# nadongjun/mirbft

Hardware: AMD Instinct MI355X
Metric: SHA-256 digests/s (request + batch digests), Actions.Hash stream (higher is better)
Workload: dtype u32

## Files before the change

### mirbft_amd/csrc/mirsha_kernels.hip

```cpp
#include <algorithm>
#include <atomic>
#include <cstdlib>
#include <cstdio>

#include <hip/hip_ext.h>

#include "mirsha_kernels.h"
#include "sha256_device.h"

namespace mirsha {

template <bool kMax>
__device__ __forceinline__ uint32_t wave_reduce(uint32_t v) {
    auto op = [](uint32_t a, uint32_t b) { return kMax ? (a > b ? a : b) : (a < b ? a : b); };
    constexpr int id = kMax ? 0 : -1;
    v = op(v, (uint32_t)__builtin_amdgcn_update_dpp(id, (int)v, 0xB1, 0xF, 0xF, false));
    v = op(v, (uint32_t)__builtin_amdgcn_update_dpp(id, (int)v, 0x4E, 0xF, 0xF, false));
    v = op(v, (uint32_t)__builtin_amdgcn_update_dpp(id, (int)v, 0x124, 0xF, 0xF, false));
    v = op(v, (uint32_t)__builtin_amdgcn_update_dpp(id, (int)v, 0x128, 0xF, 0xF, false));
    const uint32_t r0 = __builtin_amdgcn_readlane(v, 0), r1 = __builtin_amdgcn_readlane(v, 16);
    const uint32_t r2 = __builtin_amdgcn_readlane(v, 32), r3 = __builtin_amdgcn_readlane(v, 48);
    return op(op(r0, r1), op(r2, r3));
}
__device__ __forceinline__ uint32_t wave_max(uint32_t v) { return wave_reduce<true>(v); }
__device__ __forceinline__ uint32_t wave_min(uint32_t v) { return wave_reduce<false>(v); }

struct RawChunk {
    uint32_t v[5];
    uint32_t sel;
};

__device__ __forceinline__ void issue_chunk(__amdgpu_buffer_rsrc_t rsrc, uint32_t records, uint32_t o,
                                            uint32_t blk, uint32_t q, bool active, RawChunk& c) {
    const uint32_t addr = o + 64u * blk + 16u * q;
    const uint32_t a = active ? (addr & ~3u) : 0xFFFFFFE0u;
    c.sel = be_sel(addr & 3u);
    if (a + 20u <= records || !active) {
        const auto v = __builtin_amdgcn_raw_buffer_load_b128(rsrc, a, 0, 0);
        c.v[0] = v[0]; c.v[1] = v[1]; c.v[2] = v[2]; c.v[3] = v[3];
        c.v[4] = __builtin_amdgcn_raw_buffer_load_b32(rsrc, a + 16u, 0, 0);
    } else {
        asm volatile(
            "s_nop 4\n\t"
            "buffer_load_dword %0, %5, %6, 0 offen\n\t"
            "buffer_load_dword %1, %5, %6, 0 offen offset:4\n\t"
            "buffer_load_dword %2, %5, %6, 0 offen offset:8\n\t"
            "buffer_load_dword %3, %5, %6, 0 offen offset:12\n\t"
            "buffer_load_dword %4, %5, %6, 0 offen offset:16\n\t"
            "s_waitcnt vmcnt(0)"
            : "=&v"(c.v[0]), "=&v"(c.v[1]), "=&v"(c.v[2]), "=&v"(c.v[3]), "=&v"(c.v[4])
            : "v"(a), "s"(rsrc)
            : "memory");
    }
}

typedef uint32_t u32x4a4 __attribute__((ext_vector_type(4), aligned(4)));
__device__ __forceinline__ void issue_chunk_wide(const uint8_t* __restrict__ arena, uint64_t records, uint64_t o,
                                                 uint32_t blk, uint32_t q, bool active, RawChunk& c) {
    const uint64_t addr = o + 64ull * blk + 16u * q;
    const uint64_t a = addr & ~3ull;
    c.sel = be_sel((uint32_t)addr & 3u);
#pragma unroll
    for (int k = 0; k < 5; k++) c.v[k] = 0u;
    if (active) {
        const uint32_t* p = reinterpret_cast<const uint32_t*>(arena + a);
        if (a + 20u <= records) {
            const u32x4a4 v = *reinterpret_cast<const u32x4a4*>(p);
            c.v[0] = v[0]; c.v[1] = v[1]; c.v[2] = v[2]; c.v[3] = v[3];
            c.v[4] = p[4];
        } else {
#pragma unroll
            for (int k = 0; k < 5; k++)
                if (a + 4u * k + 4u <= records) c.v[k] = p[k];
        }
    }
}

__device__ __forceinline__ void pad_words(uint32_t p, uint32_t L, bool last_block, uint32_t q, uint32_t out[4]) {
    if (p + 16u > L) {
#pragma unroll
        for (int k = 0; k < 4; k++) {
            const int32_t t = (int32_t)(L - (p + 4u * k));
            const uint32_t sh = (uint32_t)t << 3;
            const uint32_t keep = ~(0xFFFFFFFFu >> sh);
            const uint32_t mark = 0x80000000u >> sh;
            const uint32_t part = (out[k] & keep) | mark;
            out[k] = t >= 4 ? out[k] : (t < 0 ? 0u : part);
        }
        if (last_block && q == 3u) {
            out[2] = L >> 29;
            out[3] = L << 3;
        }
    }
}

template <int kWords = 16>
__device__ __forceinline__ void pad_block_uniform(uint32_t w[16], uint32_t soff, uint32_t L, bool last) {
#pragma unroll
    for (int k = 0; k < kWords; k++) {
        const int32_t t = (int32_t)(L - (soff + 4u * k));
        const uint32_t sh = (uint32_t)t << 3;
        uint32_t keep = t >= 4 ? 0xFFFFFFFFu : (t <= 0 ? 0u : ~(0xFFFFFFFFu >> sh));
        uint32_t mark = (t >= 0 && t < 4) ? 0x80000000u >> sh : 0u;
        if (k >= 14 && last) {
            keep = 0u;
            mark = k == 14 ? L >> 29 : L << 3;
        }
        keep = __builtin_amdgcn_readfirstlane(keep);
        mark = __builtin_amdgcn_readfirstlane(mark);
        w[k] = (w[k] & keep) | mark;
    }
}

__device__ __forceinline__ void finish_chunk(const RawChunk& c, uint32_t p, uint32_t L, bool last_block,
                                             uint32_t q, uint32_t out[4]) {
#pragma unroll
    for (int k = 0; k < 4; k++) out[k] = be_word(c.v[k + 1], c.v[k], c.sel);
    pad_words(p, L, last_block, q, out);
}

__device__ __forceinline__ uint32_t lds_slot(uint32_t m, uint32_t q) {
    return m * 4u + (q ^ ((m >> 2) & 3u));
}

__device__ __forceinline__ void store_digest(uint8_t* out, uint32_t msg, const uint32_t st[8]) {
    uint4* d = reinterpret_cast<uint4*>(out + 32ull * msg);
    d[0] = make_uint4(__builtin_bswap32(st[0]), __builtin_bswap32(st[1]), __builtin_bswap32(st[2]),
                      __builtin_bswap32(st[3]));
    d[1] = make_uint4(__builtin_bswap32(st[4]), __builtin_bswap32(st[5]), __builtin_bswap32(st[6]),
                      __builtin_bswap32(st[7]));
}

__device__ __forceinline__ void store_digest_buf(__amdgpu_buffer_rsrc_t ors, uint32_t msg, const uint32_t st[8]) {
    __builtin_amdgcn_raw_buffer_store_b128(
        (uint32_t __attribute__((ext_vector_type(4)))){__builtin_bswap32(st[0]), __builtin_bswap32(st[1]),
                                                        __builtin_bswap32(st[2]), __builtin_bswap32(st[3])},
        ors, 32u * msg, 0, 0);
    __builtin_amdgcn_raw_buffer_store_b128(
        (uint32_t __attribute__((ext_vector_type(4)))){__builtin_bswap32(st[4]), __builtin_bswap32(st[5]),
                                                        __builtin_bswap32(st[6]), __builtin_bswap32(st[7])},
        ors, 32u * msg + 16u, 0, 0);
}

constexpr int kSc1 = 1 << 4;

__device__ __forceinline__ void store_digest_sc1(__amdgpu_buffer_rsrc_t ors, uint32_t msg, const uint32_t st[8]) {
    __builtin_amdgcn_raw_buffer_store_b128(
        (uint32_t __attribute__((ext_vector_type(4)))){__builtin_bswap32(st[0]), __builtin_bswap32(st[1]),
                                                        __builtin_bswap32(st[2]), __builtin_bswap32(st[3])},
        ors, 32u * msg, 0, kSc1);
    __builtin_amdgcn_raw_buffer_store_b128(
        (uint32_t __attribute__((ext_vector_type(4)))){__builtin_bswap32(st[4]), __builtin_bswap32(st[5]),
                                                        __builtin_bswap32(st[6]), __builtin_bswap32(st[7])},
        ors, 32u * msg + 16u, 0, kSc1);
}

constexpr uint32_t kPrioTop = 3;
__device__ __forceinline__ void progress_prio(uint32_t blk) {
    blk = (uint32_t)__builtin_amdgcn_readfirstlane((int)blk);
    const uint32_t p = blk < kPrioTop ? kPrioTop - blk : 0u;
    if (p >= 3u) __builtin_amdgcn_s_setprio(3);
    else if (p == 2u) __builtin_amdgcn_s_setprio(2);
    else if (p == 1u) __builtin_amdgcn_s_setprio(1);
    else __builtin_amdgcn_s_setprio(0);
}

constexpr uint32_t kPrioProgress = 4;
__device__ __forceinline__ void fixed_prio(uint32_t p) {
    p = (uint32_t)__builtin_amdgcn_readfirstlane((int)p);
    if (p >= 3u) __builtin_amdgcn_s_setprio(3);
    else if (p == 2u) __builtin_amdgcn_s_setprio(2);
    else if (p == 1u) __builtin_amdgcn_s_setprio(1);
    else __builtin_amdgcn_s_setprio(0);
}

constexpr uint32_t kPrioBalance = 5;
constexpr uint32_t kBalDone = 0xFFFFFFFFu;
__shared__ uint32_t g_bal_prog[4 * 16];

__device__ __forceinline__ uint32_t lds_addr(const void* p) {
    return (uint32_t)(size_t)(const __attribute__((address_space(3))) void*)p;
}
__device__ __forceinline__ uint32_t lds_load_nodma(const uint32_t* p) {
    uint32_t v;
    asm volatile("ds_read_b32 %0, %1\n\ts_waitcnt lgkmcnt(0)" : "=v"(v) : "v"(lds_addr(p)) : "memory");
    return v;
}

__shared__ uint32_t g_simd_live[4];
constexpr uint32_t kLoneSeen = 0xFFFFFFFFu;
__device__ __forceinline__ bool simd_alone(uint32_t sel) {
    if (sel == 0u || sel == kLoneSeen) return sel != 0u;
    const uint32_t n = lds_load_nodma(&g_simd_live[sel - 1u]);
    return (uint32_t)__builtin_amdgcn_readfirstlane((int)n) <= 1u;
}
__device__ __forceinline__ uint32_t bal_word() {
    uint32_t hw;
    asm volatile("s_getreg_b32 %0, hwreg(HW_REG_HW_ID)" : "=s"(hw));
    return ((hw >> 4) & 3u) * 16u + (hw & 15u);
}
__device__ __forceinline__ void balance_prio(uint32_t blk) {
    const uint32_t me = bal_word();
    __hip_atomic_store(g_bal_prog + me, blk, __ATOMIC_RELAXED, __HIP_MEMORY_SCOPE_WORKGROUP);
    const uint32_t* row = g_bal_prog + (me & ~15u);
    uint32_t ahead = 0;
#pragma unroll
    for (uint32_t k = 0; k < 16; k++)
        ahead += __hip_atomic_load(row + k, __ATOMIC_RELAXED, __HIP_MEMORY_SCOPE_WORKGROUP) < blk ? 1u : 0u;
    fixed_prio(3u - min(3u, (uint32_t)__builtin_amdgcn_readfirstlane((int)ahead)));
}
__device__ __forceinline__ void balance_done() {
    __hip_atomic_store(g_bal_prog + bal_word(), kBalDone, __ATOMIC_RELAXED, __HIP_MEMORY_SCOPE_WORKGROUP);
}

template <bool kNoYield>
__device__ __forceinline__ void hash_tile_pipelined(__amdgpu_buffer_rsrc_t rsrc, const uint32_t vo[4],
                                                    const uint32_t sel[4], uint32_t L, uint32_t min_l, bool uni,
                                                    bool tail_ok, const TailWords& tw, uint32_t wave_nb,
                                                    uint32_t loop_nb, uint32_t nb, uint32_t lane, uint4* my,
                                                    uint32_t st[8]) {
    const uint32_t q = lane & 3u;
    uint32_t nx[4][4];
    auto load_raw = [&](uint32_t blk) {
#pragma unroll
        for (int j = 0; j < 4; j++) {
            const auto v = __builtin_amdgcn_raw_buffer_load_b128(rsrc, vo[j], 64u * blk, 0);
            nx[j][0] = v[0]; nx[j][1] = v[1]; nx[j][2] = v[2]; nx[j][3] = v[3];
        }
    };
    auto write_tile = [&](uint32_t blk) {
        const uint32_t soff = 64u * blk;
        const bool pad = soff + 64u > min_l;
#pragma unroll
        for (int j = 0; j < 4; j++) {
            uint32_t wq[4];
#pragma unroll
            for (int k = 0; k < 4; k++) wq[k] = be_word(k < 3 ? nx[j][k + 1] : 0u, nx[j][k], sel[j]);
            if (pad && !uni) {
                const uint32_t Lm = (uint32_t)__shfl((int)L, 16 * j + (int)(lane >> 2), 64);
                pad_words(soff + 16u * q, Lm, blk + 1u == blocks_for_len(Lm), q, wq);
            }
            my[lds_slot(16u * j + (lane >> 2), q)] = make_uint4(wq[0], wq[1], wq[2], wq[3]);
        }
        __builtin_amdgcn_fence(__ATOMIC_RELEASE, "wavefront");
        __builtin_amdgcn_wave_barrier();
        __builtin_amdgcn_fence(__ATOMIC_ACQUIRE, "wavefront");
    };
    auto read_tile = [&](uint32_t w[16]) {
#pragma unroll
        for (int k = 0; k < 4; k++) {
            const uint4 x = my[lds_slot(lane, (uint32_t)k)];
            w[4 * k + 0] = x.x; w[4 * k + 1] = x.y; w[4 * k + 2] = x.z; w[4 * k + 3] = x.w;
        }
        __builtin_amdgcn_fence(__ATOMIC_RELEASE, "wavefront");
        __builtin_amdgcn_wave_barrier();
        __builtin_amdgcn_fence(__ATOMIC_ACQUIRE, "wavefront");
    };
    auto pad_uniform = [&](uint32_t blk, uint32_t w[16]) {
        if (64u * blk + 64u > min_l && uni) {
            uint32_t wnb;
            asm volatile("s_mov_b32 %0, %1" : "=s"(wnb) : "s"(wave_nb));
            pad_block_uniform(w, 64u * blk, min_l, wnb - blk == 1u);
        }
    };
    uint32_t w[16];
    load_raw(0u);
    write_tile(0u);
    if (1u < wave_nb) load_raw(1u);
    read_tile(w);
    for (uint32_t blk = 0; blk < loop_nb; blk++) {
        pad_uniform(blk, w);
        const bool next = blk + 1u < wave_nb;
        uint32_t wn[16];
        progress_prio(blk);
        compress_asm_hooked<kNoYield>(st, w, blk < nb, [&](int k) {
            if (k == 0 && next) {
                write_tile(blk + 1u);
                if (blk + 2u < wave_nb) load_raw(blk + 2u);
            } else if (k == 2 && next) {
                read_tile(wn);
            }
        });
#pragma unroll
        for (int i = 0; i < 16; i++) w[i] = wn[i];
    }
    if (tail_ok) {
        const uint32_t blk = wave_nb - 1u;
        pad_block_uniform<4>(w, 64u * blk, min_l, false);
        progress_prio(blk);
        if (blk < nb) compress_asm_tail(st, w, tw);
    }
}

constexpr uint32_t kTilePaused = 0, kTileDone = 1;
template <bool kLds, bool kWide, bool kFused = false, bool kPf = false, bool kNoYield = false, bool kDma = false,
          bool kDmaPipe = false, int kDiag = 0>
__device__ __forceinline__ uint32_t hash_tile(const uint8_t* __restrict__ arena, uint64_t arena_len,
                                          const uint64_t* __restrict__ off, const uint32_t* __restrict__ len,
                                          const uint32_t* __restrict__ order, uint32_t n, uint8_t* __restrict__ out,
                                          uint4* my, uint32_t t, uint32_t lane, uint32_t fprio = 0,
                                          uint32_t b0 = 0u, uint32_t b1 = 0xFFFFFFFFu, uint32_t* st_io = nullptr,
                                          uint32_t lone_sel = 0u, uint4* my2 = nullptr,
                                          unsigned long long* lone_tr = nullptr) {
    auto block_prio = [&](uint32_t blk) {
        if constexpr (kDiag == 2) {
            return;
        } else if constexpr (kFused) {
            if (fprio == kPrioBalance)
                balance_prio(blk);
            else if (fprio == kPrioProgress)
                progress_prio(blk);
            else
                fixed_prio(fprio);
        } else {
            progress_prio(blk);
        }
    };
    __builtin_amdgcn_s_setprio(3);
    const uint32_t slot = t * 64u + lane;
    const bool valid = slot < n;
    const uint32_t slot_c = valid ? slot : n - 1u;
    const uint32_t msg = order ? order[slot_c] : slot_c;
    const uint32_t L_ = len[msg];
    const uint64_t o_ = off[msg];
    const uint32_t L = valid ? L_ : 0u;
    const uint64_t o = valid ? o_ : 0u;
    const uint32_t nb = valid ? blocks_for_len(L) : 0u;
    const uint32_t max_l = wave_max(valid ? L : 0u);
    const uint32_t wave_nb = blocks_for_len(max_l);

    const uint64_t records = (arena_len + 3u) & ~3ull;
    const __amdgpu_buffer_rsrc_t rsrc =
        __builtin_amdgcn_make_buffer_rsrc((void*)arena, (short)0, (int)(uint32_t)records, 0x00020000);
    auto issue = [&](uint64_t mo, uint32_t blk, uint32_t q, bool active, RawChunk& rc) {
        if constexpr (kWide)
            issue_chunk_wide(arena, records, mo, blk, q, active, rc);
        else
            issue_chunk(rsrc, (uint32_t)records, (uint32_t)mo, blk, q, active, rc);
    };

    uint32_t st[8];
#pragma unroll
    for (int i = 0; i < 8; i++) st[i] = (st_io && b0) ? st_io[i] : kH0[i];
    const bool finished = b1 >= wave_nb;

    if constexpr (kLds && !kWide) {
        const uint32_t q = lane & 3u;
        const uint64_t reach = valid ? o + 64ull * wave_nb + 20u : 0ull;
        const bool far = __builtin_amdgcn_ballot_w64(reach > records) == 0;
        const bool aligned = __builtin_amdgcn_ballot_w64(valid && (o & 3u) != 0u) == 0;
        const uint32_t min_l = wave_min(valid ? L : 0xFFFFFFFFu);
        const bool uni = max_l == min_l;
        const int32_t u_last = (int32_t)(min_l - 64u * (wave_nb - 1u));
        const bool tail_ok = uni && u_last <= 16;
        const TailWords tw = tail_words(u_last, min_l);
        uint32_t vo[4], sel[4];
#pragma unroll
        for (int j = 0; j < 4; j++) {
            const uint32_t a = (uint32_t)__shfl((int)(uint32_t)o, 16 * j + (int)(lane >> 2), 64) + 16u * q;
            vo[j] = a & ~3u;
            sel[j] = be_sel(a & 3u);
        }
        auto stage = [&](uint32_t blk, uint32_t w[16], uint32_t ln, bool trim) {
            const uint32_t soff = 64u * blk;
            const uint32_t qq = ln & 3u;
            const bool skip = trim && soff + 16u * qq >= min_l;
            RawChunk rc[4];
            if (far && !trim) {
#pragma unroll
                for (int j = 0; j < 4; j++) {
                    const auto v = __builtin_amdgcn_raw_buffer_load_b128(rsrc, vo[j], soff, 0);
                    rc[j].v[0] = v[0]; rc[j].v[1] = v[1]; rc[j].v[2] = v[2]; rc[j].v[3] = v[3];
                    rc[j].v[4] = 0u;
                }
                if (!aligned) {
#pragma unroll
                    for (int j = 0; j < 4; j++)
                        rc[j].v[4] = __builtin_amdgcn_raw_buffer_load_b32(rsrc, vo[j], soff + 16u, 0);
                }
            } else if (far) {
#pragma unroll
                for (int j = 0; j < 4; j++) {
                    const uint32_t a = skip ? 0xFFFFFFE0u : vo[j] + soff;
                    const auto v = __builtin_amdgcn_raw_buffer_load_b128(rsrc, a, 0, 0);
                    rc[j].v[0] = v[0]; rc[j].v[1] = v[1]; rc[j].v[2] = v[2]; rc[j].v[3] = v[3];
                    rc[j].v[4] = aligned ? 0u : __builtin_amdgcn_raw_buffer_load_b32(rsrc, a + 16u, 0, 0);
                }
            } else {
#pragma unroll
                for (int j = 0; j < 4; j++)
                    issue_chunk(rsrc, (uint32_t)records, vo[j] + soff, 0u, 0u, !skip, rc[j]);
            }
            const bool pad = soff + 64u > min_l;
#pragma unroll
            for (int j = 0; j < 4; j++) {
                uint32_t wq[4];
#pragma unroll
                for (int k = 0; k < 4; k++) wq[k] = be_word(rc[j].v[k + 1], rc[j].v[k], sel[j]);
                if (pad && !uni) {
                    const uint32_t Lm = (uint32_t)__shfl((int)L, 16 * j + (int)(ln >> 2), 64);
                    pad_words(soff + 16u * qq, Lm, blk + 1u == blocks_for_len(Lm), qq, wq);
                }
                my[lds_slot(16u * j + (ln >> 2), qq)] = make_uint4(wq[0], wq[1], wq[2], wq[3]);
            }
            __builtin_amdgcn_fence(__ATOMIC_RELEASE, "wavefront");
            __builtin_amdgcn_wave_barrier();
            __builtin_amdgcn_fence(__ATOMIC_ACQUIRE, "wavefront");
#pragma unroll
            for (int k = 0; k < 4; k++) {
                const uint4 x = my[lds_slot(ln, (uint32_t)k)];
                w[4 * k + 0] = x.x; w[4 * k + 1] = x.y; w[4 * k + 2] = x.z; w[4 * k + 3] = x.w;
            }
            __builtin_amdgcn_fence(__ATOMIC_RELEASE, "wavefront");
            __builtin_amdgcn_wave_barrier();
            __builtin_amdgcn_fence(__ATOMIC_ACQUIRE, "wavefront");
        };
        const uint32_t loop_nb = tail_ok ? wave_nb - 1u : wave_nb;
        if constexpr (kPf && !kDma && !kDmaPipe) {
            if (far && aligned && b0 == 0u && finished) {
                hash_tile_pipelined<kNoYield>(rsrc, vo, sel, L, min_l, uni, tail_ok, tw, wave_nb, loop_nb, nb, lane, my,
                                              st);
                goto digest;
            }
        }
        const uint32_t loop_end = min(loop_nb, b1);
        bool dma = false;
        if constexpr (kFused || kDma || kDmaPipe) dma = far && aligned;
        if (dma) {
            const uint32_t qd = (lane & 3u) ^ ((lane >> 4) & 3u);
            uint32_t vd[4];
#pragma unroll
            for (int j = 0; j < 4; j++)
                vd[j] = (uint32_t)__shfl((int)(uint32_t)o, 16 * j + (int)(lane >> 2), 64) + 16u * qd;
            const bool deep = kFused && my2 != nullptr;
            auto tile_of = [&](uint32_t blk) { return (deep && (blk & 1u)) ? my2 : my; };
            auto issue_dma = [&](uint32_t blk) {
                if constexpr (kDiag == 1) return;
                uint4* t = tile_of(blk);
#pragma unroll
                for (int j = 0; j < 4; j++)
                    __builtin_amdgcn_raw_ptr_buffer_load_lds(
                        rsrc, (__attribute__((address_space(3))) void*)(t + 64 * j), 16, vd[j], 64u * blk, 0, 0);
            };
            const uint32_t d0 = (uint32_t)__builtin_amdgcn_readfirstlane((int)b0);
            const uint32_t d1 = (uint32_t)__builtin_amdgcn_readfirstlane((int)loop_end);
            const uint32_t dmin = (uint32_t)__builtin_amdgcn_readfirstlane((int)min_l);
            auto read_words = [&](uint32_t x[16]) {
                asm volatile("s_waitcnt vmcnt(0)" ::: "memory");
#pragma unroll
                for (int k = 0; k < 4; k++) {
                    const uint4 v = my[lds_slot(lane, (uint32_t)k)];
                    x[4 * k + 0] = v.x; x[4 * k + 1] = v.y; x[4 * k + 2] = v.z; x[4 * k + 3] = v.w;
                }
            };
            auto finish_words = [&](uint32_t blk, uint32_t x[16]) {
#pragma unroll
                for (int k = 0; k < 16; k++) x[k] = __builtin_bswap32(x[k]);
                if (64u * blk + 64u > dmin) {
                    uint32_t wnb;
                    asm volatile("s_mov_b32 %0, %1" : "=s"(wnb) : "s"(wave_nb));
                    if (uni) {
                        pad_block_uniform(x, 64u * blk, dmin, wnb - blk == 1u);
                    } else {
#pragma unroll
                        for (int k = 0; k < 4; k++)
                            pad_words(64u * blk + 16u * (uint32_t)k, L, blk + 1u == nb, (uint32_t)k, &x[4 * k]);
                    }
                }
            };
            if constexpr (kDmaPipe) {
                if (d0 < d1) {
                    uint32_t w[16];
                    issue_dma(d0);
                    read_words(w);
                    asm volatile("s_waitcnt lgkmcnt(0)" ::: "memory");
                    if (d0 + 1u < d1) issue_dma(d0 + 1u);
                    for (uint32_t blk = d0; blk < d1; blk++) {
                        finish_words(blk, w);
                        block_prio(blk);
                        const bool next = blk + 1u < d1, next2 = blk + 2u < d1;
                        uint32_t wn[16];
                        compress_asm_hooked(st, w, blk < nb, [&](int k) {
                            if (k == 2 && next) {
                                read_words(wn);
                            } else if (k == 4 && next) {
                                asm volatile("s_waitcnt lgkmcnt(0)" ::: "memory");
                                if (next2) issue_dma(blk + 2u);
                            }
                        });
#pragma unroll
                        for (int i = 0; i < 16; i++) w[i] = wn[i];
                    }
                }
            }
            if (!kDmaPipe && d0 < d1) {
                issue_dma(d0);
                if (deep && d0 + 1u < d1) issue_dma(d0 + 1u);
            }
            for (uint32_t blk = kDmaPipe ? d1 : d0; blk < d1; blk++) {
                const uint32_t soff = 64u * blk;
                if (deep && blk + 1u < d1)
                    asm volatile("s_waitcnt vmcnt(4)" ::: "memory");
                else
                    asm volatile("s_waitcnt vmcnt(0)" ::: "memory");
                if constexpr (kFused) block_prio(blk);
                uint32_t w[16];
                const uint4* tb = tile_of(blk);
#pragma unroll
                for (int k = 0; k < 4; k++) {
                    const uint4 x = tb[lds_slot(lane, (uint32_t)k)];
                    w[4 * k + 0] = x.x; w[4 * k + 1] = x.y; w[4 * k + 2] = x.z; w[4 * k + 3] = x.w;
                }
                asm volatile("s_waitcnt lgkmcnt(0)" ::: "memory");
                if (blk + (deep ? 2u : 1u) < d1) issue_dma(blk + (deep ? 2u : 1u));
#pragma unroll
                for (int k = 0; k < 16; k++) w[k] = __builtin_bswap32(w[k]);
                if (soff + 64u > dmin) {
                    uint32_t wnb;
                    asm volatile("s_mov_b32 %0, %1" : "=s"(wnb) : "s"(wave_nb));
                    if (uni) {
                        pad_block_uniform(w, soff, dmin, wnb - blk == 1u);
                    } else {
#pragma unroll
                        for (int k = 0; k < 4; k++)
                            pad_words(soff + 16u * (uint32_t)k, L, blk + 1u == nb, (uint32_t)k, &w[4 * k]);
                    }
                }
                if constexpr (!kFused) block_prio(blk);
                if constexpr (kFused) {
                    if (lone_sel != 0u && simd_alone(lone_sel)) lone_sel = kLoneSeen;
                    if (lone_sel == kLoneSeen) {
                        if (lone_tr != nullptr) {
                            if (lane == 0u) *lone_tr |= 1ull << 63 | (unsigned long long)min(blk, 1023u) << 53;
                            lone_tr = nullptr;
                        }
                        if (blk < nb) compress_asm_lat(st, w);
                    } else if (blk < nb) {
                        compress_asm(st, w);
                    }
                } else if (blk < nb) {
                    compress_asm(st, w);
                }
            }
        }
        for (uint32_t blk = dma ? loop_end : b0; blk < loop_end; blk++) {
            const uint32_t soff = 64u * blk;
            uint32_t w[16];
            stage(blk, w, lane, false);
            if (soff + 64u > min_l && uni) {
                uint32_t wnb;
                asm volatile("s_mov_b32 %0, %1" : "=s"(wnb) : "s"(wave_nb));
                pad_block_uniform(w, soff, min_l, wnb - blk == 1u);
            }
            block_prio(blk);
            if (blk < nb) compress_asm(st, w);
        }
        if (tail_ok && finished) {
            const uint32_t blk = wave_nb - 1u;
            uint32_t w[16];
            uint32_t ln;
            asm volatile("v_mov_b32 %0, %1" : "=v"(ln) : "v"(lane));
            stage(blk, w, ln, true);
            pad_block_uniform<4>(w, 64u * blk, min_l, false);
            block_prio(blk);
            if (blk < nb) compress_asm_tail(st, w, tw);
        }
    } else if constexpr (kLds) {
        const uint32_t q = lane & 3u;
        uint32_t Lj[4], nbj[4];
        uint64_t oj[4];
#pragma unroll
        for (int j = 0; j < 4; j++) {
            const int src = 16 * j + (int)(lane >> 2);
            Lj[j] = (uint32_t)__shfl((int)L, src, 64);
            oj[j] = (uint64_t)(uint32_t)__shfl((int)(uint32_t)o, src, 64);
            oj[j] |= (uint64_t)(uint32_t)__shfl((int)(uint32_t)(o >> 32), src, 64) << 32;
            nbj[j] = (uint32_t)__shfl((int)nb, src, 64);
        }
        for (uint32_t blk = 0; blk < wave_nb; blk++) {
            RawChunk rc[4];
#pragma unroll
            for (int j = 0; j < 4; j++) issue(oj[j], blk, q, blk < nbj[j], rc[j]);
#pragma unroll
            for (int j = 0; j < 4; j++) {
                uint32_t wq[4];
                finish_chunk(rc[j], 64u * blk + 16u * q, Lj[j], blk + 1u == nbj[j], q, wq);
                my[lds_slot(16u * j + (lane >> 2), q)] = make_uint4(wq[0], wq[1], wq[2], wq[3]);
            }
            __builtin_amdgcn_fence(__ATOMIC_RELEASE, "wavefront");
            __builtin_amdgcn_wave_barrier();
            __builtin_amdgcn_fence(__ATOMIC_ACQUIRE, "wavefront");
            uint32_t w[16];
#pragma unroll
            for (int k = 0; k < 4; k++) {
                const uint4 x = my[lds_slot(lane, (uint32_t)k)];
                w[4 * k + 0] = x.x; w[4 * k + 1] = x.y; w[4 * k + 2] = x.z; w[4 * k + 3] = x.w;
            }
            __builtin_amdgcn_fence(__ATOMIC_RELEASE, "wavefront");
            __builtin_amdgcn_wave_barrier();
            __builtin_amdgcn_fence(__ATOMIC_ACQUIRE, "wavefront");
            progress_prio(blk);
            if (blk < nb) compress_asm(st, w);
        }
    } else {
        for (uint32_t blk = 0; blk < wave_nb; blk++) {
            const bool active = blk < nb;
            RawChunk rc[4];
#pragma unroll
            for (int q = 0; q < 4; q++) issue(o, blk, (uint32_t)q, active, rc[q]);
            uint32_t w[16];
#pragma unroll
            for (int q = 0; q < 4; q++)
                finish_chunk(rc[q], 64u * blk + 16u * q, L, blk + 1u == nb, (uint32_t)q, &w[4 * q]);
            progress_prio(blk);
            if (active) compress_asm(st, w);
        }
    }
digest:
    if (!finished) {
#pragma unroll
        for (int i = 0; i < 8; i++) st_io[i] = st[i];
        return kTilePaused;
    }
    if (valid) {
        if constexpr (kFused) {
            const __amdgpu_buffer_rsrc_t ors =
                __builtin_amdgcn_make_buffer_rsrc((void*)out, (short)0, (int)(32u * n), 0x00020000);
            store_digest_sc1(ors, msg, st);
        } else if constexpr (kLds && !kWide) {
            const __amdgpu_buffer_rsrc_t ors =
                __builtin_amdgcn_make_buffer_rsrc((void*)out, (short)0, (int)(32u * n), 0x00020000);
            store_digest_buf(ors, msg, st);
        } else {
            store_digest(out, msg, st);
        }
    }
    return kTileDone;
}

constexpr uint32_t kMsgWaves = 1;
constexpr uint32_t kMsgOcc = 8, kTileSlots = 256;
template <bool kLds, bool kWide = false>
__global__ __launch_bounds__(64 * kMsgWaves, kWide ? 6 : kMsgOcc) void sha256_msgs_kernel(
    const uint8_t* __restrict__ arena, uint64_t arena_len, const uint64_t* __restrict__ off,
    const uint32_t* __restrict__ len, const uint32_t* __restrict__ order, uint32_t n,
    uint8_t* __restrict__ out) {
    __shared__ uint4 tile[kMsgWaves][kTileSlots];
    const uint32_t lane = threadIdx.x & 63u;
    const uint32_t wv = threadIdx.x >> 6;
    const uint32_t t = blockIdx.x * kMsgWaves + wv;
    if (t * 64u >= n) return;
    hash_tile<kLds, kWide>(arena, arena_len, off, len, order, n, out, tile[wv], t, lane);
}

constexpr uint32_t kCuLds = 96u * 1024u;
template <int kMode>
__global__ __launch_bounds__(1024, 1) void sha256_msgs_cu_kernel(const uint8_t* __restrict__ arena,
                                                                 uint64_t arena_len,
                                                                 const uint64_t* __restrict__ off,
                                                                 const uint32_t* __restrict__ len,
                                                                 const uint32_t* __restrict__ order, uint32_t n,
                                                                 uint8_t* __restrict__ out) {
    extern __shared__ uint4 cu_lds[];
    const uint32_t lane = threadIdx.x & 63u;
    const uint32_t wv = threadIdx.x >> 6;
    const uint32_t t = blockIdx.x * (blockDim.x >> 6) + wv;
    if (t * 64u >= n) return;
    hash_tile<true, false, false, true, kMode == 1, kMode == 0 || kMode >= 4, kMode == 3,
              kMode == 4 ? 1 : kMode == 5 ? 2 : 0>(arena, arena_len, off, len, order, n, out, cu_lds + 256u * wv, t,
                                                     lane);
}

__device__ __forceinline__ uint32_t ld_u32(__amdgpu_buffer_rsrc_t rs, uint32_t off, bool live);
__device__ __forceinline__ void load_digest(__amdgpu_buffer_rsrc_t rsrc, uint32_t id, bool live, uint4& x0,
                                            uint4& x1);
__device__ __forceinline__ void overlap_chain(const uint8_t* __restrict__ digests, uint32_t n_digests,
                                              const uint32_t* __restrict__ cidx, uint32_t n_entries,
                                              const uint32_t* __restrict__ cfirst, uint32_t n_lists,
                                              uint8_t* __restrict__ list_out, uint32_t g, uint32_t lane,
                                              uint32_t prio_mode) {
    __builtin_amdgcn_s_setprio(3);
    const uint32_t k = g * 64u + lane;
    const bool valid = k < n_lists;
    const uint32_t kc = valid ? k : n_lists - 1u;
    const uint32_t e0_ = cfirst[kc], e1_ = cfirst[kc + 1];
    const uint32_t e0 = valid ? e0_ : 0u;
    const uint32_t c = valid ? e1_ - e0_ : 0u;
    const uint32_t L = 32u * c;
    const uint32_t nb = valid ? blocks_for_len(L) : 0u;
    const uint32_t wave_nb = blocks_for_len(32u * wave_max(c));
    const __amdgpu_buffer_rsrc_t drs =
        __builtin_amdgcn_make_buffer_rsrc((void*)digests, (short)0, (int)(32u * n_digests), 0x00020000);
    const __amdgpu_buffer_rsrc_t irs =
        __builtin_amdgcn_make_buffer_rsrc((void*)cidx, (short)0, (int)(4u * n_entries), 0x00020000);
    uint32_t st[8];
#pragma unroll
    for (int i = 0; i < 8; i++) st[i] = kH0[i];
    uint32_t i0 = ld_u32(irs, 4u * e0, 0u < c), i1 = ld_u32(irs, 4u * (e0 + 1u), 1u < c);
    for (uint32_t blk = 0; blk < wave_nb; blk++) {
        const uint32_t d0 = 2u * blk;
        uint4 x[4];
        load_digest(drs, i0, d0 < c, x[0], x[1]);
        load_digest(drs, i1, d0 + 1u < c, x[2], x[3]);
        i0 = ld_u32(irs, 4u * (e0 + d0 + 2u), d0 + 2u < c);
        i1 = ld_u32(irs, 4u * (e0 + d0 + 3u), d0 + 3u < c);
        uint32_t w[16];
#pragma unroll
        for (int half = 0; half < 2; half++) {
            const uint32_t di = d0 + (uint32_t)half;
            const uint4 a = x[2 * half], b = x[2 * half + 1];
            w[8 * half + 0] = __builtin_bswap32(a.x) | (di == c ? 0x80000000u : 0u);
            w[8 * half + 1] = __builtin_bswap32(a.y); w[8 * half + 2] = __builtin_bswap32(a.z);
            w[8 * half + 3] = __builtin_bswap32(a.w); w[8 * half + 4] = __builtin_bswap32(b.x);
            w[8 * half + 5] = __builtin_bswap32(b.y); w[8 * half + 6] = __builtin_bswap32(b.z);
            w[8 * half + 7] = __builtin_bswap32(b.w);
        }
        if (blk + 1u == nb) {
            w[14] = L >> 29;
            w[15] = L << 3;
        }
        fixed_prio(prio_mode == 0u   ? 3u - min(3u, 4u * blk / wave_nb)
                   : prio_mode == 1u ? 3u - min(3u, blk)
                   : prio_mode == 2u ? 3u
                                     : 1u);
        if (blk < nb) compress_asm(st, w);
    }
    if (valid) {
        const __amdgpu_buffer_rsrc_t ors =
            __builtin_amdgcn_make_buffer_rsrc((void*)list_out, (short)0, (int)(32u * n_lists), 0x00020000);
        store_digest_buf(ors, k, st);
    }
}

constexpr uint32_t kOverlapOcc = 7;
__global__ __launch_bounds__(64, kOverlapOcc) void sha256_msgs_overlap_kernel(OverlapArgs a) {
    __shared__ uint4 tile[kTileSlots];
    const uint32_t lane = threadIdx.x;
    if (blockIdx.x < a.list_waves) {
        overlap_chain(a.prev_digests, a.n_req_prev, a.cidx, a.n_entries, a.cfirst, a.n_lists, a.list_out,
                      blockIdx.x, lane, a.chain_prio);
        return;
    }
    const uint32_t t = blockIdx.x - a.list_waves;
    if (t * 64u >= a.n_req) return;
    hash_tile<true, false>(a.arena, a.arena_len, a.off, a.len, a.order, a.n_req, a.req_out, tile, t, lane);
}

__global__ __launch_bounds__(kBlockThreads) void sha256_msgs_lowocc_kernel(
    const uint8_t* __restrict__ arena, uint64_t arena_len, const uint64_t* __restrict__ off,
    const uint32_t* __restrict__ len, const uint32_t* __restrict__ order, uint32_t n, uint8_t* __restrict__ out) {
    const uint32_t lane = threadIdx.x & 63u;
    const uint32_t t = blockIdx.x * kWavesPerBlock + (threadIdx.x >> 6);
    if (t * 64u >= n) return;
    const uint32_t slot = t * 64u + lane;
    const bool valid = slot < n;
    const uint32_t msg = valid ? (order ? order[slot] : slot) : 0u;
    const uint32_t L = valid ? len[msg] : 0u;
    const uint32_t o = valid ? (uint32_t)off[msg] : 0u;
    const uint32_t nb = valid ? blocks_for_len(L) : 0u;
    const uint32_t wave_nb = wave_max(nb);
    const uint32_t records = (uint32_t)((arena_len + 3u) & ~3ull);
    const __amdgpu_buffer_rsrc_t rsrc =
        __builtin_amdgcn_make_buffer_rsrc((void*)arena, (short)0, (int)records, 0x00020000);
    uint32_t st[8];
#pragma unroll
    for (int i = 0; i < 8; i++) st[i] = kH0[i];
    RawChunk cur[4];
#pragma unroll
    for (int q = 0; q < 4; q++) issue_chunk(rsrc, records, o, 0u, (uint32_t)q, 0u < nb, cur[q]);
    for (uint32_t blk = 0; blk < wave_nb; blk++) {
        RawChunk nxt[4];
#pragma unroll
        for (int q = 0; q < 4; q++) issue_chunk(rsrc, records, o, blk + 1u, (uint32_t)q, blk + 1u < nb, nxt[q]);
        uint32_t w[16];
#pragma unroll
        for (int q = 0; q < 4; q++)
            finish_chunk(cur[q], 64u * blk + 16u * q, L, blk + 1u == nb, (uint32_t)q, &w[4 * q]);
        if (blk < nb) compress_asm_lat(st, w);
#pragma unroll
        for (int q = 0; q < 4; q++) cur[q] = nxt[q];
    }
    if (valid) store_digest(out, msg, st);
}

constexpr uint32_t kPairThreads = 128;

struct PairRing {
    uint4 kw[2][16][64];
};

__device__ __forceinline__ void produce_kw(uint32_t w[16], uint4 (*slot)[64], uint32_t lane) {
#pragma unroll
    for (int q = 0; q < 16; q++) {
        uint32_t kw[4];
#pragma unroll
        for (int i = 0; i < 4; i++) {
            const int j = 4 * q + i;
            if (j >= 16) w[j & 15] += ssig1(w[(j - 2) & 15]) + w[(j - 7) & 15] + ssig0(w[(j - 15) & 15]);
            kw[i] = kK[j] + w[j & 15];
        }
        slot[q][lane] = make_uint4(kw[0], kw[1], kw[2], kw[3]);
    }
}

__device__ __forceinline__ void consume_kw(uint4 (*slot)[64], uint32_t lane, uint32_t st[8], bool live) {
    uint32_t s[8];
#pragma unroll
    for (int i = 0; i < 8; i++) s[i] = st[i];
    uint4 a = slot[0][lane], b = slot[1][lane];
#pragma unroll
    for (int c = 0; c < 8; c++) {
        uint4 na = a, nb = b;
        if (c < 7) {
            na = slot[2 * c + 2][lane];
            nb = slot[2 * c + 3][lane];
        }
        rounds_kw8_asm(s, a, b);
        a = na;
        b = nb;
    }
    if (live) {
#pragma unroll
        for (int i = 0; i < 8; i++) st[i] += s[i];
    }
}

__device__ __forceinline__ uint32_t ld_u32(__amdgpu_buffer_rsrc_t rs, uint32_t off, bool live);
__device__ __forceinline__ void load_digest(__amdgpu_buffer_rsrc_t rsrc, uint32_t id, bool live, uint4& x0,
                                            uint4& x1);

struct ArenaBlocks {
    __amdgpu_buffer_rsrc_t rsrc;
    uint32_t records, o, L, nb;
    RawChunk cur[4];
    __device__ void start(const uint8_t* arena, uint64_t arena_len, uint32_t off_, uint32_t L_, uint32_t nb_) {
        records = (uint32_t)((arena_len + 3u) & ~3ull);
        rsrc = __builtin_amdgcn_make_buffer_rsrc((void*)arena, (short)0, (int)records, 0x00020000);
        o = off_;
        L = L_;
        nb = nb_;
#pragma unroll
        for (int q = 0; q < 4; q++) issue_chunk(rsrc, records, o, 0u, (uint32_t)q, 0u < nb, cur[q]);
    }
    __device__ void block(uint32_t blk, uint32_t w[16]) {
        RawChunk nxt[4];
#pragma unroll
        for (int q = 0; q < 4; q++) issue_chunk(rsrc, records, o, blk + 1u, (uint32_t)q, blk + 1u < nb, nxt[q]);
#pragma unroll
        for (int q = 0; q < 4; q++) finish_chunk(cur[q], 64u * blk + 16u * q, L, blk + 1u == nb, (uint32_t)q, &w[4 * q]);
#pragma unroll
        for (int q = 0; q < 4; q++) cur[q] = nxt[q];
    }
};

struct ListBlocks {
    __amdgpu_buffer_rsrc_t drs, irs;
    uint32_t e0, c, L, nb;
    uint4 cur[4];
    uint32_t nx0, nx1;
    __device__ void start(const uint8_t* digests, uint32_t n_digests, const uint32_t* cidx, uint32_t n_entries,
                          uint32_t e0_, uint32_t c_, uint32_t nb_) {
        drs = __builtin_amdgcn_make_buffer_rsrc((void*)digests, (short)0, (int)(32u * n_digests), 0x00020000);
        irs = __builtin_amdgcn_make_buffer_rsrc((void*)cidx, (short)0, (int)(4u * n_entries), 0x00020000);
        e0 = e0_;
        c = c_;
        L = 32u * c;
        nb = nb_;
        nx0 = ld_u32(irs, 4u * (e0 + 2u), 2u < c);
        nx1 = ld_u32(irs, 4u * (e0 + 3u), 3u < c);
        const uint32_t i0 = ld_u32(irs, 4u * e0, 0u < c), i1 = ld_u32(irs, 4u * (e0 + 1u), 1u < c);
        load_digest(drs, i0, 0u < c, cur[0], cur[1]);
        load_digest(drs, i1, 1u < c, cur[2], cur[3]);
    }
    __device__ void block(uint32_t blk, uint32_t w[16]) {
        uint4 nxt[4];
        load_digest(drs, nx0, 2u * blk + 2u < c, nxt[0], nxt[1]);
        load_digest(drs, nx1, 2u * blk + 3u < c, nxt[2], nxt[3]);
        const uint32_t nn0 = ld_u32(irs, 4u * (e0 + 2u * blk + 4u), 2u * blk + 4u < c);
        const uint32_t nn1 = ld_u32(irs, 4u * (e0 + 2u * blk + 5u), 2u * blk + 5u < c);
#pragma unroll
        for (int half = 0; half < 2; half++) {
            const uint32_t di = 2u * blk + (uint32_t)half;
            const uint4 x0 = cur[2 * half], x1 = cur[2 * half + 1];
            w[8 * half + 0] = __builtin_bswap32(x0.x) | (di == c ? 0x80000000u : 0u);
            w[8 * half + 1] = __builtin_bswap32(x0.y); w[8 * half + 2] = __builtin_bswap32(x0.z);
            w[8 * half + 3] = __builtin_bswap32(x0.w); w[8 * half + 4] = __builtin_bswap32(x1.x);
            w[8 * half + 5] = __builtin_bswap32(x1.y); w[8 * half + 6] = __builtin_bswap32(x1.z);
            w[8 * half + 7] = __builtin_bswap32(x1.w);
        }
        if (blk + 1u == nb) {
            w[14] = L >> 29;
            w[15] = L << 3;
        }
#pragma unroll
        for (int i = 0; i < 4; i++) cur[i] = nxt[i];
        nx0 = nn0;
        nx1 = nn1;
    }
};

template <class Src>
__device__ __forceinline__ void pair_loop(Src& src, PairRing& ring, bool producer, uint32_t lane, uint32_t nb,
                                          uint32_t st[8]) {
    const uint32_t wave_nb = wave_max(nb);
#pragma unroll
    for (int i = 0; i < 8; i++) st[i] = kH0[i];
    if (producer && wave_nb) {
        uint32_t w[16];
        src.block(0u, w);
        produce_kw(w, ring.kw[0], lane);
    }
    __syncthreads();
    for (uint32_t blk = 0; blk < wave_nb; blk++) {
        if (producer) {
            if (blk + 1u < wave_nb) {
                uint32_t w[16];
                src.block(blk + 1u, w);
                produce_kw(w, ring.kw[(blk + 1u) & 1u], lane);
            }
        } else {
            consume_kw(ring.kw[blk & 1u], lane, st, blk < nb);
// ... 1256 lines not shown
```

### mirbft_amd/csrc/sha256_device.h

```cpp
#pragma once
#include <hip/hip_runtime.h>
#include <stdint.h>

#include "sha256_rounds_asm.h"

namespace mirsha {

static constexpr uint32_t kK[64] = {
    0x428a2f98u, 0x71374491u, 0xb5c0fbcfu, 0xe9b5dba5u, 0x3956c25bu, 0x59f111f1u, 0x923f82a4u,
    0xab1c5ed5u, 0xd807aa98u, 0x12835b01u, 0x243185beu, 0x550c7dc3u, 0x72be5d74u, 0x80deb1feu,
    0x9bdc06a7u, 0xc19bf174u, 0xe49b69c1u, 0xefbe4786u, 0x0fc19dc6u, 0x240ca1ccu, 0x2de92c6fu,
    0x4a7484aau, 0x5cb0a9dcu, 0x76f988dau, 0x983e5152u, 0xa831c66du, 0xb00327c8u, 0xbf597fc7u,
    0xc6e00bf3u, 0xd5a79147u, 0x06ca6351u, 0x14292967u, 0x27b70a85u, 0x2e1b2138u, 0x4d2c6dfcu,
    0x53380d13u, 0x650a7354u, 0x766a0abbu, 0x81c2c92eu, 0x92722c85u, 0xa2bfe8a1u, 0xa81a664bu,
    0xc24b8b70u, 0xc76c51a3u, 0xd192e819u, 0xd6990624u, 0xf40e3585u, 0x106aa070u, 0x19a4c116u,
    0x1e376c08u, 0x2748774cu, 0x34b0bcb5u, 0x391c0cb3u, 0x4ed8aa4au, 0x5b9cca4fu, 0x682e6ff3u,
    0x748f82eeu, 0x78a5636fu, 0x84c87814u, 0x8cc70208u, 0x90befffau, 0xa4506cebu, 0xbef9a3f7u,
    0xc67178f2u};

static constexpr uint32_t kH0[8] = {0x6a09e667u, 0xbb67ae85u, 0x3c6ef372u, 0xa54ff53au,
                                    0x510e527fu, 0x9b05688cu, 0x1f83d9abu, 0x5be0cd19u};

__device__ __forceinline__ uint32_t rotr(uint32_t x, int n) { return __builtin_rotateright32(x, n); }
__device__ __forceinline__ uint32_t xor3(uint32_t a, uint32_t b, uint32_t c) {
    return __builtin_amdgcn_bitop3_b32(a, b, c, 0x96);
}
__device__ __forceinline__ uint32_t bsig0(uint32_t x) { return xor3(rotr(x, 2), rotr(x, 13), rotr(x, 22)); }
__device__ __forceinline__ uint32_t bsig1(uint32_t x) { return xor3(rotr(x, 6), rotr(x, 11), rotr(x, 25)); }
__device__ __forceinline__ uint32_t ssig0(uint32_t x) { return xor3(rotr(x, 7), rotr(x, 18), x >> 3); }
__device__ __forceinline__ uint32_t ssig1(uint32_t x) { return xor3(rotr(x, 17), rotr(x, 19), x >> 10); }
__device__ __forceinline__ uint32_t ch(uint32_t e, uint32_t f, uint32_t g) { return g ^ (e & (f ^ g)); }
__device__ __forceinline__ uint32_t maj(uint32_t a, uint32_t b, uint32_t c) {
    return __builtin_amdgcn_bitop3_b32(a, b, c, 0xE8);
}

__device__ __forceinline__ void compress(uint32_t st[8], uint32_t w[16]) {
    uint32_t a = st[0], b = st[1], c = st[2], d = st[3];
    uint32_t e = st[4], f = st[5], g = st[6], h = st[7];
#define MIRSHA_ROUND(a, b, c, d, e, f, g, h, j)                                              \
    {                                                                                        \
        if ((j) >= 16)                                                                       \
            w[(j)&15] += ssig1(w[((j)-2) & 15]) + w[((j)-7) & 15] + ssig0(w[((j)-15) & 15]);  \
        uint32_t t1 = h + bsig1(e) + ch(e, f, g) + kK[(j)] + w[(j)&15];                      \
        d += t1;                                                                             \
        h = t1 + bsig0(a) + maj(a, b, c);                                                    \
    }
#pragma unroll
    for (int j = 0; j < 64; j += 8) {
        MIRSHA_ROUND(a, b, c, d, e, f, g, h, j + 0);
        MIRSHA_ROUND(h, a, b, c, d, e, f, g, j + 1);
        MIRSHA_ROUND(g, h, a, b, c, d, e, f, j + 2);
        MIRSHA_ROUND(f, g, h, a, b, c, d, e, j + 3);
        MIRSHA_ROUND(e, f, g, h, a, b, c, d, j + 4);
        MIRSHA_ROUND(d, e, f, g, h, a, b, c, j + 5);
        MIRSHA_ROUND(c, d, e, f, g, h, a, b, j + 6);
        MIRSHA_ROUND(b, c, d, e, f, g, h, a, j + 7);
    }
#undef MIRSHA_ROUND
    st[0] += a; st[1] += b; st[2] += c; st[3] += d;
    st[4] += e; st[5] += f; st[6] += g; st[7] += h;
}

__device__ __forceinline__ void compress_asm(uint32_t st[8], uint32_t w[16]) {
    uint32_t s[8];
#pragma unroll
    for (int i = 0; i < 8; i++) s[i] = st[i];
    rounds_asm(s, w);
#pragma unroll
    for (int i = 0; i < 8; i++) st[i] += s[i];
}

template <bool kNoYield = false, class H>
__device__ __forceinline__ void compress_asm_hooked(uint32_t st[8], uint32_t w[16], bool live, H hook) {
    uint32_t s[8];
#pragma unroll
    for (int i = 0; i < 8; i++) s[i] = st[i];
    if constexpr (kNoYield)
        rounds_asm_nonop(s, w, hook);
    else
        rounds_asm(s, w, hook);
#pragma unroll
    for (int i = 0; i < 8; i++) st[i] = live ? st[i] + s[i] : st[i];
}

__device__ __forceinline__ TailWords tail_words(int32_t u, uint32_t L) {
    auto sgpr = [](uint32_t x) { return (uint32_t)__builtin_amdgcn_readfirstlane((int)x); };
    TailWords k;
    k.c4 = u == 16 ? 0x80000000u : 0u;
    k.c14 = L >> 29;
    k.c15 = L << 3;
    k.kw4 = kK[4] + k.c4;
    k.kw14 = kK[14] + k.c14;
    k.kw15 = kK[15] + k.c15;
    k.cs16 = sgpr(ssig1(k.c14));
    k.cs17 = sgpr(ssig1(k.c15));
    k.cs19 = sgpr(ssig0(k.c4));
    k.cs29 = sgpr(ssig0(k.c14));
    k.cs30 = sgpr(ssig0(k.c15) + k.c14);
    return k;
}

__device__ __forceinline__ void compress_asm_tail(uint32_t st[8], uint32_t w[16], const TailWords& k) {
    uint32_t s[8];
#pragma unroll
    for (int i = 0; i < 8; i++) s[i] = st[i];
    rounds_asm_tail(s, w, k);
#pragma unroll
    for (int i = 0; i < 8; i++) st[i] += s[i];
}

__device__ __forceinline__ void compress_asm_lat(uint32_t st[8], uint32_t w[16]) {
    uint32_t s[8];
#pragma unroll
    for (int i = 0; i < 8; i++) s[i] = st[i];
    rounds_asm_nonop(s, w);
#pragma unroll
    for (int i = 0; i < 8; i++) st[i] += s[i];
}

__device__ __host__ __forceinline__ uint32_t blocks_for_len(uint32_t L) { return (L + 72u) >> 6; }

__device__ __forceinline__ uint32_t be_word(uint32_t hi, uint32_t lo, uint32_t sel) {
    return __builtin_amdgcn_perm(hi, lo, sel);
}
__device__ __forceinline__ uint32_t be_sel(uint32_t r) { return 0x00010203u + r * 0x01010101u; }

__device__ __forceinline__ void pad_chunk(uint32_t w[4], uint32_t p, uint32_t L, bool last_block,
                                          uint32_t q) {
#pragma unroll
    for (int k = 0; k < 4; k++) {
        const int64_t rem = (int64_t)L - (int64_t)(p + 4u * k);
        const uint32_t valid = rem <= 0 ? 0u : (rem >= 4 ? 4u : (uint32_t)rem);
        const uint32_t mask = valid == 4u ? 0xFFFFFFFFu : (valid == 0u ? 0u : ~(0xFFFFFFFFu >> (8u * valid)));
        uint32_t x = w[k] & mask;
        if (rem >= 0 && rem < 4) x |= 0x80u << (24u - 8u * (uint32_t)rem);
        w[k] = x;
    }
    if (last_block && q == 3u) {
        w[2] = L >> 29;
        w[3] = L << 3;
    }
}

}
```

Before: 5.081 billion.

## Add uniform-length dense-wave fast path skipping reductions and shuffles in LDS staging

When every valid lane in a wave has the same message length, the wave skips the min/max reductions and takes the length from the first lane. If the offsets are also contiguous and 4-byte aligned, per-lane addresses come from a scalar base instead of shuffles and ballots, and the unaligned fifth-word loads and mixed-length padding become separate cold branches. Tail-word setup is moved to where it is used and computed with scalar rotates instead of readfirstlane. This adds extra ballots/compares up front and more code paths, and it includes census asm markers, which look like instrumentation.

Measured after the change: 5.117 billion (median of 6 runs). Within noise of the previous version (+0.7%).

```diff
diff --git a/mirbft_amd/csrc/mirsha_kernels.hip b/mirbft_amd/csrc/mirsha_kernels.hip
--- a/mirbft_amd/csrc/mirsha_kernels.hip
+++ b/mirbft_amd/csrc/mirsha_kernels.hip
@@ -9,6 +9,8 @@
 #include "sha256_device.h"
 
 namespace mirsha {
+
+#define CENSUS_MARK(name) asm volatile("; census " name)
 
 template <bool kMax>
 __device__ __forceinline__ uint32_t wave_reduce(uint32_t v) {
@@ -158,10 +160,9 @@
 constexpr uint32_t kPrioTop = 3;
 __device__ __forceinline__ void progress_prio(uint32_t blk) {
     blk = (uint32_t)__builtin_amdgcn_readfirstlane((int)blk);
-    const uint32_t p = blk < kPrioTop ? kPrioTop - blk : 0u;
-    if (p >= 3u) __builtin_amdgcn_s_setprio(3);
-    else if (p == 2u) __builtin_amdgcn_s_setprio(2);
-    else if (p == 1u) __builtin_amdgcn_s_setprio(1);
+    if (blk + 3u <= kPrioTop) __builtin_amdgcn_s_setprio(3);
+    else if (blk + 2u == kPrioTop) __builtin_amdgcn_s_setprio(2);
+    else if (blk + 1u == kPrioTop) __builtin_amdgcn_s_setprio(1);
     else __builtin_amdgcn_s_setprio(0);
 }
 
@@ -326,7 +327,24 @@
     const uint32_t L = valid ? L_ : 0u;
     const uint64_t o = valid ? o_ : 0u;
     const uint32_t nb = valid ? blocks_for_len(L) : 0u;
-    const uint32_t max_l = wave_max(valid ? L : 0u);
+    uint32_t max_l, min_l = 0u;
+    [[maybe_unused]] uint32_t L0 = 0u;
+    [[maybe_unused]] bool same_len = false;
+    [[maybe_unused]] uint64_t vmask = 0;
+    if constexpr (kLds && !kWide) {
+        L0 = (uint32_t)__builtin_amdgcn_readfirstlane((int)L_);
+        vmask = __builtin_amdgcn_uicmp(slot, n, 36 );
+        same_len = (__builtin_amdgcn_uicmp(L_, L0, 33 ) & vmask) == 0;
+        if (same_len) {
+            max_l = min_l = L0;
+        } else {
+            CENSUS_MARK("off");
+            max_l = wave_max(L);
+            min_l = wave_min(valid ? L : 0xFFFFFFFFu);
+        }
+    } else {
+        max_l = wave_max(L);
+    }
     const uint32_t wave_nb = blocks_for_len(max_l);
 
     const uint64_t records = (arena_len + 3u) & ~3ull;
@@ -346,62 +364,104 @@
 
     if constexpr (kLds && !kWide) {
         const uint32_t q = lane & 3u;
-        const uint64_t reach = valid ? o + 64ull * wave_nb + 20u : 0ull;
-        const bool far = __builtin_amdgcn_ballot_w64(reach > records) == 0;
-        const bool aligned = __builtin_amdgcn_ballot_w64(valid && (o & 3u) != 0u) == 0;
-        const uint32_t min_l = wave_min(valid ? L : 0xFFFFFFFFu);
         const bool uni = max_l == min_l;
         const int32_t u_last = (int32_t)(min_l - 64u * (wave_nb - 1u));
         const bool tail_ok = uni && u_last <= 16;
-        const TailWords tw = tail_words(u_last, min_l);
+        bool far, aligned;
         uint32_t vo[4], sel[4];
-#pragma unroll
-        for (int j = 0; j < 4; j++) {
-            const uint32_t a = (uint32_t)__shfl((int)(uint32_t)o, 16 * j + (int)(lane >> 2), 64) + 16u * q;
-            vo[j] = a & ~3u;
-            sel[j] = be_sel(a & 3u);
+        const uint64_t o0 = (uint64_t)(uint32_t)__builtin_amdgcn_readfirstlane((int)(uint32_t)o_) |
+                            (uint64_t)(uint32_t)__builtin_amdgcn_readfirstlane((int)(uint32_t)(o_ >> 32)) << 32;
+        const uint32_t nv = (uint32_t)__builtin_popcountll(vmask);
+        bool dense = !kFused && same_len && ((uint32_t)o0 & 3u) == 0u && (nv == 1u || (L0 & 3u) == 0u);
+        if (dense) dense = (__builtin_amdgcn_uicmpl(o_, o0 + (uint64_t)lane * L0, 33 ) & vmask) == 0;
+        if (dense) {
+            const uint64_t reach = o0 + (uint64_t)(nv - 1u) * L0 + 64ull * wave_nb + 20u;
+            unsigned long long room;
+            far = !__builtin_usubll_overflow(records, reach, &room);
+            aligned = true;
+            const uint32_t a0 = (uint32_t)o0 + (lane >> 2) * L0 + 16u * q;
+#pragma unroll
+            for (int j = 0; j < 4; j++) {
+                vo[j] = a0 + 16u * (uint32_t)j * L0;
+                sel[j] = be_sel(0u);
+            }
+        } else {
+            CENSUS_MARK("off");
+            const uint64_t reach = valid ? o + 64ull * wave_nb + 20u : 0ull;
+            far = __builtin_amdgcn_ballot_w64(reach > records) == 0;
+            aligned = __builtin_amdgcn_ballot_w64(valid && (o & 3u) != 0u) == 0;
+#pragma unroll
+            for (int j = 0; j < 4; j++) {
+                const uint32_t a = (uint32_t)__shfl((int)(uint32_t)o, 16 * j + (int)(lane >> 2), 64) + 16u * q;
+                vo[j] = a & ~3u;
+                sel[j] = be_sel(a & 3u);
+            }
         }
         auto stage = [&](uint32_t blk, uint32_t w[16], uint32_t ln, bool trim) {
             const uint32_t soff = 64u * blk;
             const uint32_t qq = ln & 3u;
             const bool skip = trim && soff + 16u * qq >= min_l;
             RawChunk rc[4];
+            if (trim)
+                CENSUS_MARK("tail");
+            else
+                CENSUS_MARK("stage");
             if (far && !trim) {
 #pragma unroll
                 for (int j = 0; j < 4; j++) {
                     const auto v = __builtin_amdgcn_raw_buffer_load_b128(rsrc, vo[j], soff, 0);
                     rc[j].v[0] = v[0]; rc[j].v[1] = v[1]; rc[j].v[2] = v[2]; rc[j].v[3] = v[3];
-                    rc[j].v[4] = 0u;
                 }
                 if (!aligned) {
+                    CENSUS_MARK("off");
 #pragma unroll
                     for (int j = 0; j < 4; j++)
                         rc[j].v[4] = __builtin_amdgcn_raw_buffer_load_b32(rsrc, vo[j], soff + 16u, 0);
+                } else {
+#pragma unroll
+                    for (int j = 0; j < 4; j++) asm volatile("" : "=v"(rc[j].v[4]));
                 }
             } else if (far) {
+                uint32_t a[4];
 #pragma unroll
                 for (int j = 0; j < 4; j++) {
-                    const uint32_t a = skip ? 0xFFFFFFE0u : vo[j] + soff;
-                    const auto v = __builtin_amdgcn_raw_buffer_load_b128(rsrc, a, 0, 0);
+                    a[j] = skip ? 0xFFFFFFE0u : vo[j] + soff;
+                    const auto v = __builtin_amdgcn_raw_buffer_load_b128(rsrc, a[j], 0, 0);
                     rc[j].v[0] = v[0]; rc[j].v[1] = v[1]; rc[j].v[2] = v[2]; rc[j].v[3] = v[3];
-                    rc[j].v[4] = aligned ? 0u : __builtin_amdgcn_raw_buffer_load_b32(rsrc, a + 16u, 0, 0);
+                }
+                if (!aligned) {
+                    CENSUS_MARK("off");
+#pragma unroll
+                    for (int j = 0; j < 4; j++)
+                        rc[j].v[4] = __builtin_amdgcn_raw_buffer_load_b32(rsrc, a[j] + 16u, 0, 0);
+                } else {
+#pragma unroll
+                    for (int j = 0; j < 4; j++) asm volatile("" : "=v"(rc[j].v[4]));
                 }
             } else {
+                CENSUS_MARK("off");
 #pragma unroll
                 for (int j = 0; j < 4; j++)
                     issue_chunk(rsrc, (uint32_t)records, vo[j] + soff, 0u, 0u, !skip, rc[j]);
             }
             const bool pad = soff + 64u > min_l;
-#pragma unroll
-            for (int j = 0; j < 4; j++) {
+            auto words = [&](int j, bool mixed_pad) {
                 uint32_t wq[4];
 #pragma unroll
                 for (int k = 0; k < 4; k++) wq[k] = be_word(rc[j].v[k + 1], rc[j].v[k], sel[j]);
-                if (pad && !uni) {
+                if (mixed_pad) {
                     const uint32_t Lm = (uint32_t)__shfl((int)L, 16 * j + (int)(ln >> 2), 64);
                     pad_words(soff + 16u * qq, Lm, blk + 1u == blocks_for_len(Lm), qq, wq);
                 }
                 my[lds_slot(16u * j + (ln >> 2), qq)] = make_uint4(wq[0], wq[1], wq[2], wq[3]);
+            };
+            if (pad && !uni) {
+                CENSUS_MARK("off");
+#pragma unroll
+                for (int j = 0; j < 4; j++) words(j, true);
+            } else {
+#pragma unroll
+                for (int j = 0; j < 4; j++) words(j, false);
             }
             __builtin_amdgcn_fence(__ATOMIC_RELEASE, "wavefront");
             __builtin_amdgcn_wave_barrier();
@@ -418,6 +478,7 @@
         const uint32_t loop_nb = tail_ok ? wave_nb - 1u : wave_nb;
         if constexpr (kPf && !kDma && !kDmaPipe) {
             if (far && aligned && b0 == 0u && finished) {
+                const TailWords tw = tail_words(u_last, min_l);
                 hash_tile_pipelined<kNoYield>(rsrc, vo, sel, L, min_l, uni, tail_ok, tw, wave_nb, loop_nb, nb, lane, my,
                                               st);
                 goto digest;
@@ -548,6 +609,7 @@
             uint32_t w[16];
             stage(blk, w, lane, false);
             if (soff + 64u > min_l && uni) {
+                CENSUS_MARK("off");
                 uint32_t wnb;
                 asm volatile("s_mov_b32 %0, %1" : "=s"(wnb) : "s"(wave_nb));
                 pad_block_uniform(w, soff, min_l, wnb - blk == 1u);
@@ -563,6 +625,7 @@
             stage(blk, w, ln, true);
             pad_block_uniform<4>(w, 64u * blk, min_l, false);
             block_prio(blk);
+            const TailWords tw = tail_words(u_last, min_l);
             if (blk < nb) compress_asm_tail(st, w, tw);
         }
     } else if constexpr (kLds) {
@@ -617,6 +680,7 @@
         }
     }
 digest:
+    CENSUS_MARK("epilogue");
     if (!finished) {
 #pragma unroll
         for (int i = 0; i < 8; i++) st_io[i] = st[i];
diff --git a/mirbft_amd/csrc/sha256_device.h b/mirbft_amd/csrc/sha256_device.h
--- a/mirbft_amd/csrc/sha256_device.h
+++ b/mirbft_amd/csrc/sha256_device.h
@@ -83,8 +83,14 @@
     for (int i = 0; i < 8; i++) st[i] = live ? st[i] + s[i] : st[i];
 }
 
+__device__ __forceinline__ uint32_t rotr_scalar(uint32_t x, int n) {
+    uint32_t hi = x << (32 - n);
+    asm("" : "+s"(hi));
+    return (x >> n) | hi;
+}
 __device__ __forceinline__ TailWords tail_words(int32_t u, uint32_t L) {
-    auto sgpr = [](uint32_t x) { return (uint32_t)__builtin_amdgcn_readfirstlane((int)x); };
+    auto s0 = [](uint32_t x) { return rotr_scalar(x, 7) ^ rotr_scalar(x, 18) ^ (x >> 3); };
+    auto s1 = [](uint32_t x) { return rotr_scalar(x, 17) ^ rotr_scalar(x, 19) ^ (x >> 10); };
     TailWords k;
     k.c4 = u == 16 ? 0x80000000u : 0u;
     k.c14 = L >> 29;
@@ -92,11 +98,11 @@
     k.kw4 = kK[4] + k.c4;
     k.kw14 = kK[14] + k.c14;
     k.kw15 = kK[15] + k.c15;
-    k.cs16 = sgpr(ssig1(k.c14));
-    k.cs17 = sgpr(ssig1(k.c15));
-    k.cs19 = sgpr(ssig0(k.c4));
-    k.cs29 = sgpr(ssig0(k.c14));
-    k.cs30 = sgpr(ssig0(k.c15) + k.c14);
+    k.cs16 = s1(k.c14);
+    k.cs17 = s1(k.c15);
+    k.cs19 = s0(k.c4);
+    k.cs29 = s0(k.c14);
+    k.cs30 = s0(k.c15) + k.c14;
     return k;
 }
 
```
